# arneschneuing/DiffSBDD

Measured on AMD Instinct MI355X. Metric: sampled ligands/sec (500-step DDPM, fullatom_cond) at 1/2/4/8 MI355X, higher is better.
Workload: dtype f32

## Files before the change

### diffsbdd_amd/csrc/engine_state.h

```cpp
#pragma once

static thread_local std::string g_err;
static int fail(int code, const std::string& msg) { g_err = msg; return code; }

#define HIP_TRY(expr)                                                              \
  do {                                                                             \
    hipError_t _e = (expr);                                                        \
    if (_e != hipSuccess)                                                          \
      return fail(DSBDD_ERR_LAUNCH, std::string(#expr) + ": " + hipGetErrorString(_e)); \
  } while (0)
#define RC_TRY(expr)                       \
  do {                                     \
    const int _rc = (expr);                \
    if (_rc != DSBDD_OK) return _rc;       \
  } while (0)

struct StreamDevice {
  int prev = -1;
  bool switched = false;
  explicit StreamDevice(void* stream) {
    hipStream_t s = static_cast<hipStream_t>(stream);
    if (!s) return;
    hipDevice_t d = 0;
    int cur = 0;
// ... 113 lines not shown
  dsbdd_config cfg;
  std::vector<const float*> slots;
  bool has_weights = false;
  char* ws = nullptr;
  size_t ws_bytes = 0;
  int64_t cap_lig = 0, cap_poc = 0, cap_batch = 0, cap_edges = 0;
  bool lvl_stats_zeroed = false;
  int64_t cap_edgesL = 0;
  int prune = 1;
  int cone = 1;
  int64_t ghost_slots = 0;
  std::vector<int> plan_radius, plan_ghost;
  int plan_timed_level = kLevels - 1;
  bool frame = false;
  int64_t frame_nlig = 0, frame_npoc = 0, frame_batch = 0, frame_n3 = 0, frame_cap3 = 0;
  bool ghost_dirty = true;
  bool h0_pocket_valid = false;
  int64_t cap_tiles = 0;
  int64_t cap_tiles16 = 0;
  unsigned granule16 = 0;
  unsigned splitk = 0;
  int emu = 0;
  DerivedReady derived;
  float *trace_h = nullptr, *trace_x = nullptr;
  int n_cu = 256;
  int chain = 1;
  int64_t chain_min_rows = 0;
  int fork_front = 0;
  hipStream_t side_stream = nullptr;
  hipEvent_t ev_fork = nullptr, ev_join = nullptr;
  int level_rows = 0;
  int fold_scan = 1;
  int lig_head = 1;
  int edge_bperm = 1;
  int profile = 0;
  int64_t prof_call = 0;
  bool time_now = false;
  std::vector<hipEvent_t> ev;
  size_t ev_used = 0;
  struct GraphEntry {
    std::vector<uint64_t> key;
    int seen = 0;
    hipGraph_t graph = nullptr;
    hipGraphExec_t exec = nullptr;
    std::vector<int> plan_radius, plan_ghost;
    int plan_timed_level = 0;
    void destroy() { if (exec) (void)hipGraphExecDestroy(exec); if (graph) (void)hipGraphDestroy(graph); }
  };
  std::vector<GraphEntry> graphs;
  int use_graph = 1;
  int coord_split = 1;
  int node_group = 1;
  int edge_max_wg = 0;
  int64_t n_replay = 0, n_capture = 0, n_eager = 0;
  unsigned long long* ts_buf = nullptr;
  int ts_cap = 0, ts_next = 0;
  hipStream_t cap_stream = nullptr;
  dsbdd_engine() : Workspace{} {}
  void drop_graphs() {
    for (GraphEntry& g : graphs) g.destroy();
    graphs.clear();
  }
  void invalidate_derived() { derived = DerivedReady{}; }
  ~dsbdd_engine() {
    for (hipEvent_t e : ev) (void)hipEventDestroy(e);
    drop_graphs();
// ... 34 lines not shown
}
static int w2_pack_missing(dsbdd_engine* e, hipStream_t s) {
  const dsbdd_config& c = e->cfg;
  for (int kind = W2_KINDS - 1; kind >= 0; --kind) {
    if (!w2_enabled(e, kind) || e->derived.w2[kind]) continue;
    for (int blk = 0; blk < c.n_layers; ++blk)
      for (int which = 0; which < c.inv_sublayers + 2; ++which) {
        const float* src = which < c.inv_sublayers ? e->slots[gcl_slot(c, blk, which, DSBDD_GCL_E2_WT)]
                         : e->slots[eq_slot(c, blk, which == c.inv_sublayers ? DSBDD_EQ_C_W2T : DSBDD_EQ_X_W2T)];
        if (!src) continue;
        kW2Kinds[kind].pack(s, src, w2_copy(e, kind, blk, which), c.hidden_nf);
        HIP_TRY(hipGetLastError());
      }
    e->derived.w2[kind] = true;
  }
  return DSBDD_OK;
}

static bool env_int(const char* name, long long* v, bool mask = false) {
  const char* s = getenv(name);
  if (!s) return false;
  *v = mask ? (long long)strtoul(s, nullptr, 0) : (long long)atoi(s);
  return true;
}
static int env_int_in(const char* name, long long lo, long long hi, int dflt) {
  long long v;
  return env_int(name, &v) && v >= lo && v <= hi ? (int)v : dflt;
}
static void read_env_switches(dsbdd_engine* e) {
  long long v;
  const std::pair<const char*, int*> off_on_zero[] = {
      {"DSBDD_GRAPH", &e->use_graph}, {"DSBDD_EDGE_BPERM", &e->edge_bperm}, {"DSBDD_COORD_SPLIT", &e->coord_split},
      {"DSBDD_NODE_GROUP", &e->node_group}, {"DSBDD_PRUNE", &e->prune}, {"DSBDD_LIG_HEAD", &e->lig_head},
      {"DSBDD_NODE_CHAIN", &e->chain}};
  for (const auto& sw : off_on_zero) if (env_int(sw.first, &v) && v == 0) *sw.second = 0;
  const std::pair<const char*, int*> on_nonzero[] = {{"DSBDD_LEVEL_ROWS", &e->level_rows}, {"DSBDD_FORK", &e->fork_front}};
  for (const auto& sw : on_nonzero) if (env_int(sw.first, &v)) *sw.second = v != 0;
  if (env_int("DSBDD_FOLD_SCAN", &v)) e->fold_scan = v > 0 ? 1 : 0;
  if (env_int("DSBDD_GRANULE16", &v, true)) e->granule16 = (unsigned)v;
  if (env_int("DSBDD_SPLITK", &v, true)) e->splitk = (unsigned)v;
  if (env_int("DSBDD_EMU", &v)) e->emu = (v == 6 || v == 9) ? (int)v : 0;
  if (env_int("DSBDD_CONE", &v)) e->cone = v <= 0 ? 0 : (v >= 2 ? 2 : 1);
  if (env_int("DSBDD_NODE_CHAIN_MIN_ROWS", &v) && v >= 0) e->chain_min_rows = v;
  if (env_int("DSBDD_EDGE_MAX_WG", &v) && v > 0) e->edge_max_wg = (int)v;
}
```

### diffsbdd_amd/csrc/forward.h

```cpp
#pragma once

struct ForwardArgs {
  const float *xh_lig, *xh_pocket, *t;
  int64_t t_count;
  const int64_t *mask_lig, *mask_pocket;
  int64_t n_lig, n_pocket, batch;
  const int32_t *ext_row, *ext_col;
  int64_t ext_n_edges;
  float *eps_lig, *eps_pocket;
  int32_t* status;
};

static bool frame_applies(const dsbdd_engine* e, const ForwardArgs& a) {
  return e->frame && !e->cfg.update_pocket_coords && !a.ext_row && a.n_lig == e->frame_nlig &&
         a.n_pocket == e->frame_npoc && a.batch == e->frame_batch;
}

static Mlp2Problem residue_encoder(const dsbdd_engine* e, const ForwardArgs& a) {
  const dsbdd_config& c = e->cfg;
  const int r = c.residue_nf, J = c.joint_nf, JP = pad4(J + 1);
  const float* const* W = e->slots.data();
  return Mlp2Problem{a.xh_pocket + 3, 3 + r, r, W[DSBDD_G_RES_ENC_W0T], pad4(2 * r), W[DSBDD_G_RES_ENC_B0], 2 * r,
                     W[DSBDD_G_RES_ENC_W1T], pad4(J), W[DSBDD_G_RES_ENC_B1], J, e->h0 + (size_t)a.n_lig * JP, JP,
                     (int)a.n_pocket};
// ... 141 lines not shown
      }
    }
    HIP_TRY(nl(sa, e->h0, JP, JP, nullptr, 0, 0, W[DSBDD_G_EMB_WT], H, W[DSBDD_G_EMB_B], nullptr, 0, e->h, H, N, H, 0));
    if (split0) {
      hipLaunchKernelGGL(gather_rows_kernel, dim3((e->frame_n3 + 3) / 4), dim3(kThreads), 0, sa, e->h + (size_t)N * H,
                         (const float*)(e->h + (size_t)nlig * H), (const int*)e->frame_rows, (int)e->frame_n3, H);
      HIP_TRY(hipGetLastError());
    }
    if (fork) HIP_TRY(hipEventRecord(e->ev_join, sa));
    return DSBDD_OK;
  }

  int edge_list() {
    if (ext) {
      HIP_TRY(zero_async(e->deg, (size_t)N * 4, s));
      if (ext_n_edges > 0) {
        hipLaunchKernelGGL(ext_edges_kernel, dim3((int)((ext_n_edges + 255) / 256)), dim3(256), 0, s, ext_row,
                           ext_col, (int)ext_n_edges, (const float*)e->x, e->erow, e->ecol, e->ed0, e->deg);
        HIP_TRY(hipGetLastError());
      }
      hipLaunchKernelGGL(scan_kernel, dim3(1), dim3(1024), 0, s, (const int*)e->deg, e->row_ptr, N, SegAlign{},
                         (const int*)nullptr, (int*)nullptr, SegAlign{});
      HIP_TRY(hipGetLastError());
      edge_bound = ext_n_edges > 0 ? ext_n_edges : 1;
      if (subset) {
        hipLaunchKernelGGL(ext_flags_init_kernel, dim3((N + 255) / 256), dim3(256), 0, s, e->act_flag, nlig, N);
        HIP_TRY(hipGetLastError());
        if (ext_n_edges > 0) {
          hipLaunchKernelGGL(ext_flags_kernel, dim3((int)((ext_n_edges + 255) / 256)), dim3(256), 0, s, ext_row,
                             ext_col, (int)ext_n_edges, nlig, e->act_flag);
          HIP_TRY(hipGetLastError());
        }
      }
    } else {
      EdgeList2 l2{e->deg2, e->row_ptr2, e->erow2, e->ecol2, e->ed02, (int)e->cap_edges,
                   SegAlign{e->node_batch, e->lig_off, e->poc_off, nlig, B, e->scan_tmp2, e->seg_base2}};
      int rc = build_edges_impl(s, e->x, nlig, N, B, c, e->node_batch, e->lig_off, e->poc_off, e->deg,
                                e->row_ptr, e->erow, e->ecol, e->ed0, e->cap_edges, status,
                                subset ? e->act_flag : nullptr, e->scan_tmp, e->seg_base,
                                split0 ? &l2 : nullptr, 0, prune ? e->lvl : nullptr);
      if (rc) return rc;
      if (prune) {
        LevelArgs la{e->node_batch, e->lig_off, e->poc_off, nlig, B, e->lvl, e->deg, e->row_ptr, e->erow, e->ecol,
                     e->ed0, e->seg_rows, e->seg_edges, e->node_base, e->edge_base, e->lvl_cnt, e->lvl_end,
                     e->lvl_list, e->row_ptrL, e->erowL, e->ecolL, e->ed0L, (int)e->cap_edgesL, e->lvl_stats,
                     n_ghost, (int)ghost_slots, (int)e->cap_edges, nullptr, nullptr};
        mean_in_levels = e->fold_scan && n_mlp == 2;
        if (mean_in_levels) { la.mean_x = e->x; la.mean_out = e->mean; }
        if (!e->lvl_stats_zeroed) {
          HIP_TRY(zero_async(e->lvl_stats, 128, s));
          e->lvl_stats_zeroed = true;
        }
        hipLaunchKernelGGL(levels_kernel, dim3(B), dim3(kThreads), 0, s, la);
        HIP_TRY(hipGetLastError());
        if (!e->fold_scan) {
          hipLaunchKernelGGL(level_scan_kernel, dim3(1), dim3(1024), 0, s, la, N);
          HIP_TRY(hipGetLastError());
        }
        hipLaunchKernelGGL(level_place_kernel, dim3(B), dim3(kThreads), 0, s, la, e->fold_scan ? 1 : 0);
        HIP_TRY(hipGetLastError());
        int64_t cb = (e->cap_edges + 255) / 256;
        if (cb > 2048) cb = 2048;
        if (cb < 1) cb = 1;
        hipLaunchKernelGGL(level_copy_kernel, dim3((int)cb), dim3(256), 0, s, la, N);
        HIP_TRY(hipGetLastError());
      }
// ... 218 lines not shown
    const bool csk = ((e->splitk >> (16 + (blk & 15))) & 1u) && can_sk;
    const bool c16 = ((e->granule16 >> (16 + (blk & 15))) & 1u) && !e->emu && !csk;
    ea.xagg_stride = (size_t)N * 3; ea.xhead_stride = (size_t)(c16 ? e->cap_tiles16 : e->cap_tiles) * 4;
    ea.tile_ctr = e->tile_ctr; ea.norm_factor = c.normalization_factor;
    ea.pass_split = (c16 || csk) ? 1 : e->coord_split;
    if (e->ts_buf && e->ts_next < e->ts_cap) ea.ts = e->ts_buf + (size_t)(e->ts_next++) * 1024;
    HIP_TRY(launch_edge(e, s, MODE_COORD, ea, L_bound(), c16, csk));
    const int n_q = ((e->coord_split || c16 || csk) && n_mlp == 2) ? 2 : 1;
    const int c_shift = c16 ? 4 : 5, c_max = (int)(c16 ? e->cap_tiles16 : e->cap_tiles) - 1;
    const bool next_mean = subset && n_mlp == 2 && blk + 1 < c.n_layers;
    if (!subset) {
      if (n_upd > 0) {
        hipLaunchKernelGGL(coord_update_kernel, dim3((3 * n_upd + 255) / 256), dim3(256), 0, s, e->x,
                           (const float*)e->xagg, (const float*)e->xagg_head, n_q, ea.xagg_stride, ea.xhead_stride,
                           L_ptr, (const int*)e->deg, 3 * n_upd, c_max, c_shift);
        HIP_TRY(hipGetLastError());
      }
    } else if (n_upd > 0 || next_mean) {
      hipLaunchKernelGGL(coord_update_mean_kernel, dim3(B), dim3(kThreads), 0, s, e->x, (const float*)e->xagg,
                         (const float*)e->xagg_head, n_q, ea.xagg_stride, ea.xhead_stride, L_ptr,
                         (const int*)e->deg, n_upd, (const int*)e->lig_off, (const int*)e->poc_off, nlig,
                         next_mean ? e->mean : (float*)nullptr, c_max, c_shift);
      HIP_TRY(hipGetLastError());
    }
    return DSBDD_OK;
  }

  int output_head() {
    LigHeadArgs lh{e->h, H, W[DSBDD_G_EMBOUT_WT], JP, W[DSBDD_G_EMBOUT_B], J,
                   W[DSBDD_G_ATOM_DEC_W0T], pad4(2 * a), W[DSBDD_G_ATOM_DEC_B0], 2 * a,
                   W[DSBDD_G_ATOM_DEC_W1T], pad4(a), W[DSBDD_G_ATOM_DEC_B1], a,
                   e->x, e->x_in, nlig, N, eps_lig, dl, status};
    if (e->lig_head && !eps_pocket && !c.update_pocket_coords && lig_head_fits(lh)) {
      HIP_TRY(launch_lig_head(s, lh));
      return DSBDD_OK;
    }
    HIP_TRY(nl(s, e->h, H, H, nullptr, 0, 0, W[DSBDD_G_EMBOUT_WT], JP, W[DSBDD_G_EMBOUT_B], nullptr, 0, e->hout, JP,
               eps_pocket ? N : n_lig, JP, 0));
    {
      Mlp2Problem dec[2] = {
          {e->hout, JP, J, W[DSBDD_G_ATOM_DEC_W0T], pad4(2 * a), W[DSBDD_G_ATOM_DEC_B0], 2 * a,
           W[DSBDD_G_ATOM_DEC_W1T], pad4(a), W[DSBDD_G_ATOM_DEC_B1], a, eps_lig + 3, dl, (int)n_lig},
          {e->hout + (size_t)n_lig * JP, JP, J, W[DSBDD_G_RES_DEC_W0T], pad4(2 * r), W[DSBDD_G_RES_DEC_B0], 2 * r,
           W[DSBDD_G_RES_DEC_W1T], pad4(r), W[DSBDD_G_RES_DEC_B1], r, eps_pocket ? eps_pocket + 3 : nullptr, dp,
           (int)n_pocket}};
      if (mlp2_fits(dec[0]) && mlp2_fits(dec[1])) {
        HIP_TRY(launch_mlp2(s, dec, eps_pocket ? 2 : 1));
      } else {
        HIP_TRY(nl(s, e->hout, JP, J, nullptr, 0, 0, W[DSBDD_G_ATOM_DEC_W0T], pad4(2 * a), W[DSBDD_G_ATOM_DEC_B0], nullptr, 0,
                   e->enc_tmp, LE, n_lig, 2 * a, 1));
        HIP_TRY(nl(s, e->enc_tmp, LE, 2 * a, nullptr, 0, 0, W[DSBDD_G_ATOM_DEC_W1T], pad4(a), W[DSBDD_G_ATOM_DEC_B1], nullptr, 0,
                   eps_lig + 3, dl, n_lig, a, 0));
        if (eps_pocket) {
          float* tmp_p = e->enc_tmp + (size_t)n_lig * LE;
          HIP_TRY(nl(s, e->hout + (size_t)n_lig * JP, JP, J, nullptr, 0, 0, W[DSBDD_G_RES_DEC_W0T], pad4(2 * r),
                     W[DSBDD_G_RES_DEC_B0], nullptr, 0, tmp_p, LE, n_pocket, 2 * r, 1));
          HIP_TRY(nl(s, tmp_p, LE, 2 * r, nullptr, 0, 0, W[DSBDD_G_RES_DEC_W1T], pad4(r), W[DSBDD_G_RES_DEC_B1], nullptr, 0,
                     eps_pocket + 3, dp, n_pocket, r, 0));
        }
      }
    }
    hipLaunchKernelGGL(finalize_kernel, dim3(B), dim3(kThreads), 0, s, (const float*)e->x, (const float*)e->x_in,
                       (const int*)e->lig_off, (const int*)e->poc_off, nlig, c.update_pocket_coords, eps_lig, dl,
                       eps_pocket, dp, status);
    HIP_TRY(hipGetLastError());
    return DSBDD_OK;
  }
// ... 28 lines not shown
```

### diffsbdd_amd/csrc/graph.h

```cpp
#pragma once
#include "common.h"

namespace dsbdd {

constexpr int kTileCtrInts = 32;
constexpr int kEdgeAlign = 32;
constexpr int kLevels = 5;

struct Cutoffs {
  int has_l, has_p, has_i;
  float cl, cp, ci;
};

__device__ __forceinline__ int lower_bound_i64(const int64_t* a, int n, int64_t v) {
  int lo = 0, hi = n;
  while (lo < hi) {
    const int mid = (lo + hi) >> 1;
    if (a[mid] < v) lo = mid + 1; else hi = mid;
  }
  return lo;
}

__global__ void prep_kernel(const int64_t* mask_lig, int n_lig, const int64_t* mask_poc, int n_poc,
                            int B, int* node_batch, int* lig_off, int* poc_off, int* tile_ctr) {
// ... 178 lines not shown
    } else {
#pragma unroll
      for (int k = 0; k < 4; ++k) if (i0 + k < n) { out[i0 + k] = run; run += v[k]; }
    }
    carry += tile_total;
    __syncthreads();
  }
  if (t == 0) out[n] = carry;
  if (!seg.seg_base) return;
  __syncthreads();
  const int S = 2 * seg.B;
  auto seg_begin = [&](int k) { return k < seg.B ? seg.lig_off[k] : seg.n_lig + seg.poc_off[k - seg.B]; };
  auto seg_end = [&](int k) { return k < seg.B ? seg.lig_off[k + 1] : seg.n_lig + seg.poc_off[k - seg.B + 1]; };
  carry = 0;
  for (int base = 0; base < S; base += 1024) {
    const int k = base + t;
    int len = 0;
    if (k < S) len = (max(out[seg_end(k)] - out[seg_begin(k)], 0) + kEdgeAlign - 1) & ~(kEdgeAlign - 1);
    const int ex = carry + block_scan_1024(len, s_wave, s_carry_p);
    if (k < S) seg.seg_base[k] = ex;
    carry += s_carry;
    __syncthreads();
  }
  if (t == 0) {
    seg.seg_base[S] = carry;
    row_ptr[n] = carry;
  }
}

__device__ __forceinline__ void sample_mean_body(const float* x, const int* lig_off, const int* poc_off, int n_lig,
                                                 float* mean, float (*red)[kThreads]) {
  const int b = blockIdx.x, t = threadIdx.x;
  const int l0 = lig_off[b], l1 = lig_off[b + 1], p0 = n_lig + poc_off[b], p1 = n_lig + poc_off[b + 1];
  float s0 = 0.f, s1 = 0.f, s2 = 0.f;
  for (int i = l0 + t; i < l1; i += kThreads) { s0 += x[3 * i]; s1 += x[3 * i + 1]; s2 += x[3 * i + 2]; }
  for (int i = p0 + t; i < p1; i += kThreads) { s0 += x[3 * i]; s1 += x[3 * i + 1]; s2 += x[3 * i + 2]; }
  red[0][t] = s0; red[1][t] = s1; red[2][t] = s2;
  __syncthreads();
  for (int o = kThreads / 2; o > 0; o >>= 1) {
    if (t < o) { red[0][t] += red[0][t + o]; red[1][t] += red[1][t + o]; red[2][t] += red[2][t + o]; }
    __syncthreads();
  }
  if (t < 3) {
    int cnt = (l1 - l0) + (p1 - p0);
    if (cnt == 0) cnt = 1;
    mean[3 * b + t] = red[t][0] / (float)cnt;
  }
  __syncthreads();
}

struct LevelArgs {
  const int* node_batch; const int* lig_off; const int* poc_off; int n_lig; int B;
  int* lvl;
  const int* deg;
  const int* row_ptr_nat;
  const int* erow_nat; const int* ecol_nat; const float* ed0_nat;
  int* seg_rows;
  int* seg_edges;
  int* node_base;
  int* edge_base;
  int* lvl_cnt;
  int* lvl_end;
  int* lvl_list;
  int* row_ptr;
  int* erow; int* ecol; float* ed0; int e_cap;
  unsigned long long* stats;
  int node_off; int edge_off;
  int e_cap_nat;
  const float* mean_x; float* mean_out;
};
// ... 120 lines not shown
    for (int i = l0 + lane; i < l1; i += 64) {
      a.lvl_list[nb + (i - l0)] = i;
      a.row_ptr[i] = eb + (a.row_ptr_nat[i] - s0);
    }
    pads(eb + a.seg_edges[b]);
  }
  const int L = w + 1;
  if (L >= kLevels) return;
  const int p0 = a.n_lig + a.poc_off[b], p1 = a.n_lig + a.poc_off[b + 1];
  int n_run, e_run;
  if (fold_scan) level_bases(a, L * a.B + b, lane, n_run, e_run);
  else { n_run = a.node_base[L * a.B + b]; e_run = a.edge_base[L * a.B + b]; }
  for (int i0 = p0; i0 < p1; i0 += 64) {
    const int i = i0 + lane;
    const bool mine = i < p1 && a.lvl[i] == L;
    const int d = mine ? a.deg[i] : 0;
    const unsigned long long m = __ballot(mine);
    int incl = d;
#pragma unroll
    for (int o = 1; o < 64; o <<= 1) {
      const int u = __shfl_up(incl, o);
      if (lane >= o) incl += u;
    }
    if (mine) {
      a.lvl_list[n_run + __popcll(m & ((1ull << lane) - 1ull))] = i;
      a.row_ptr[i] = e_run + incl - d;
    }
    n_run += __popcll(m);
    e_run += __shfl(incl, 63);
  }
  pads(e_run);
}

__global__ void ghost_setup_kernel(const int* erow3, const int* ecol3, const float* ed03, const int* row_ptr3,
                                   const int* deg3, int n3, int id_src, int id_dst, int* erow, int* ecol,
                                   float* ed0, int e_cap, int* deg, int* row_ptr, int* lvl_list,
                                   const float* xframe, float* x) {
  const int total = min(row_ptr3[n3], e_cap);
  for (int p = blockIdx.x * blockDim.x + threadIdx.x; p < total; p += gridDim.x * blockDim.x) {
    const int r = erow3[p];
    erow[p] = r < 0 ? -1 : r - id_src + id_dst;
    ecol[p] = r < 0 ? 0 : ecol3[p] - id_src + id_dst;
    ed0[p] = ed03[p];
  }
  for (int i = blockIdx.x * blockDim.x + threadIdx.x; i < n3; i += gridDim.x * blockDim.x) {
    deg[id_dst + i] = deg3[i];
    row_ptr[id_dst + i] = row_ptr3[i];
    lvl_list[i] = id_dst + i;
    x[3 * (id_dst + i)] = xframe[3 * i]; x[3 * (id_dst + i) + 1] = xframe[3 * i + 1];
    x[3 * (id_dst + i) + 2] = xframe[3 * i + 2];
  }
}

__global__ __launch_bounds__(kThreads) void gather_rows_kernel(float* dst, const float* src, const int* rows, int n,
                                                               int H) {
  const int i = (blockIdx.x * kThreads + threadIdx.x) >> 6, lane = threadIdx.x & 63;
  if (i >= n) return;
  const float* a = src + (size_t)rows[i] * H;
  float* b = dst + (size_t)i * H;
  for (int k = 4 * lane; k < H; k += 256) *reinterpret_cast<float4*>(b + k) = ld4(a + k);
}

__global__ __launch_bounds__(kThreads) void canon_fill_kernel(float* h, const int* lvl, const int* twin_local,
                                                              int n_lig, int n_nodes, int ghost_base, int lo,
                                                              int hi, int H, float* pq = nullptr, int ldpq = 0) {
  const int i = n_lig + ((blockIdx.x * kThreads + threadIdx.x) >> 6), lane = threadIdx.x & 63;
// ... 221 lines not shown
```

### diffsbdd_amd/csrc/lig_head.h

```cpp
#pragma once
#include "common.h"

namespace dsbdd {

struct LigHeadArgs {
  const float* h; int H;
  const float* WoT; int ldo; const float* bo; int J;
  const float* W0T; int ld0; const float* b0; int n_hid;
  const float* W1T; int ld1; const float* b1; int n_out;
  const float* x; const float* x_in; int n_lig; int n_nodes;
  float* eps_lig; int dl; int* status;
};

constexpr int kHeadRows = 16;
constexpr int kHeadKC = 32;

__global__ __launch_bounds__(kThreads) void lig_head_kernel(LigHeadArgs p) {
  __shared__ __attribute__((aligned(16))) float sH[kHeadRows * 256];
  __shared__ float sO[kHeadRows * 128];
  __shared__ float sW[kHeadKC * 128];
  __shared__ float sD[kHeadRows * 64];
  const int t = threadIdx.x;
  const int r0 = blockIdx.x * kHeadRows;
  const int nr = min(kHeadRows, p.n_lig - r0);
// ... 53 lines not shown
    if (r >= nr) continue;
    float a = 0.f;
    for (int j = 0; j < p.n_hid; ++j) a = fmaf(sD[r * 64 + j], p.W1T[(size_t)j * p.ld1 + c], a);
    p.eps_lig[(size_t)(r0 + r) * p.dl + 3 + c] = a + p.b1[c];
  }
  bool nan = false;
  if (t < 3 * nr) {
    const int r = t / 3, k = t - 3 * r;
    const float v = p.x[3 * (size_t)(r0 + r) + k] - p.x_in[3 * (size_t)(r0 + r) + k];
    nan = v != v;
    p.eps_lig[(size_t)(r0 + r) * p.dl + k] = v;
  }
  {
    const int n_poc3 = 3 * (p.n_nodes - p.n_lig);
    const int per = (n_poc3 + gridDim.x - 1) / gridDim.x;
    const int lo = 3 * p.n_lig + blockIdx.x * per, hi = min(lo + per, 3 * p.n_nodes);
    for (int i = lo + t; i < hi; i += kThreads) {
      const float v = p.x[i] - p.x_in[i];
      nan = nan || (v != v);
    }
  }
  if (nan) atomicOr(p.status, 1);
}

inline bool lig_head_fits(const LigHeadArgs& a) {
  return a.H % kHeadKC == 0 && a.H <= 256 && a.J <= 128 && a.n_hid <= 64 && a.n_out <= 64 && a.n_lig > 0;
}

inline hipError_t launch_lig_head(hipStream_t s, const LigHeadArgs& a) {
  hipLaunchKernelGGL(lig_head_kernel, dim3((a.n_lig + kHeadRows - 1) / kHeadRows), dim3(kThreads), 0, s, a);
  return hipGetLastError();
}

}
```

Measured before the change: 38.69.

## Fuse per-sample edge build and level pruning into two front kernels; add lig_head2

Adds a per-sample path, used when pruning is on, that builds the radius graph in two block-per-sample kernels (count, then fill). The coordinates are staged in LDS, and level assignment, degree counting, segment prefix sums, level lists and padding are all computed in those kernels, replacing the longer sequence of build_edges and level kernels. It also adds a variant ligand output head that uses 8-row tiles, keeps the small MLP weights in LDS and register-prefetches the output weights. The aim is fewer launches and less global round-tripping per denoising step, at the cost of one block per sample with 1024 threads, which could underuse the GPU for small batches, and of heavy LDS use.

```diff
diff --git a/diffsbdd_amd/csrc/engine_state.h b/diffsbdd_amd/csrc/engine_state.h
--- a/diffsbdd_amd/csrc/engine_state.h
+++ b/diffsbdd_amd/csrc/engine_state.h
@@ -169,6 +169,8 @@
   int level_rows = 0;
   int fold_scan = 1;
   int lig_head = 1;
+  int front = 1;
+  int front_parts = 2;
   int edge_bperm = 1;
   int profile = 0;
   int64_t prof_call = 0;
@@ -269,11 +271,12 @@
   const std::pair<const char*, int*> off_on_zero[] = {
       {"DSBDD_GRAPH", &e->use_graph}, {"DSBDD_EDGE_BPERM", &e->edge_bperm}, {"DSBDD_COORD_SPLIT", &e->coord_split},
       {"DSBDD_NODE_GROUP", &e->node_group}, {"DSBDD_PRUNE", &e->prune}, {"DSBDD_LIG_HEAD", &e->lig_head},
-      {"DSBDD_NODE_CHAIN", &e->chain}};
+      {"DSBDD_NODE_CHAIN", &e->chain}, {"DSBDD_FRONT", &e->front}};
   for (const auto& sw : off_on_zero) if (env_int(sw.first, &v) && v == 0) *sw.second = 0;
   const std::pair<const char*, int*> on_nonzero[] = {{"DSBDD_LEVEL_ROWS", &e->level_rows}, {"DSBDD_FORK", &e->fork_front}};
   for (const auto& sw : on_nonzero) if (env_int(sw.first, &v)) *sw.second = v != 0;
   if (env_int("DSBDD_FOLD_SCAN", &v)) e->fold_scan = v > 0 ? 1 : 0;
+  if (env_int("DSBDD_FRONT_PARTS", &v, true)) e->front_parts = (int)(v & 3);
   if (env_int("DSBDD_GRANULE16", &v, true)) e->granule16 = (unsigned)v;
   if (env_int("DSBDD_SPLITK", &v, true)) e->splitk = (unsigned)v;
   if (env_int("DSBDD_EMU", &v)) e->emu = (v == 6 || v == 9) ? (int)v : 0;
diff --git a/diffsbdd_amd/csrc/forward.h b/diffsbdd_amd/csrc/forward.h
--- a/diffsbdd_amd/csrc/forward.h
+++ b/diffsbdd_amd/csrc/forward.h
@@ -197,6 +197,31 @@
           HIP_TRY(hipGetLastError());
         }
       }
+    } else if (prune && e->front && (e->front_parts & 1)) {
+      FrontArgs fa{};
+      fa.x = e->x; fa.n_nodes = N; fa.cut = cutoffs_of(c);
+      fa.deg = e->deg; fa.act_flag = e->act_flag;
+      fa.row_ptr = e->row_ptr; fa.erow = e->erow; fa.ecol = e->ecol; fa.ed0 = e->ed0; fa.e_cap = (int)e->cap_edges;
+      fa.seg_tot = e->node_base; fa.seg_base = e->seg_base;
+      if (split0)
+        fa.l2 = EdgeList2{e->deg2, e->row_ptr2, e->erow2, e->ecol2, e->ed02, (int)e->cap_edges,
+                          SegAlign{e->node_batch, e->lig_off, e->poc_off, nlig, B, e->scan_tmp2, e->seg_base2}};
+      fa.seg_tot2 = e->edge_base;
+      fa.lv = LevelArgs{e->node_batch, e->lig_off, e->poc_off, nlig, B, e->lvl, e->deg, e->row_ptr, e->erow, e->ecol,
+                        e->ed0, e->seg_rows, e->seg_edges, e->node_base, e->edge_base, e->lvl_cnt, e->lvl_end,
+                        e->lvl_list, e->row_ptrL, e->erowL, e->ecolL, e->ed0L, (int)e->cap_edgesL, e->lvl_stats,
+                        n_ghost, (int)ghost_slots, (int)e->cap_edges, nullptr, nullptr};
+      fa.status = status;
+      mean_in_levels = n_mlp == 2;
+      if (mean_in_levels) { fa.lv.mean_x = e->x; fa.lv.mean_out = e->mean; }
+      if (!e->lvl_stats_zeroed) {
+        HIP_TRY(zero_async(e->lvl_stats, 128, s));
+        e->lvl_stats_zeroed = true;
+      }
+      hipLaunchKernelGGL(front_count_kernel, dim3(B), dim3(kFrontThreads), 0, s, fa);
+      HIP_TRY(hipGetLastError());
+      hipLaunchKernelGGL(front_fill_kernel, dim3(B), dim3(kFrontThreads), 0, s, fa);
+      HIP_TRY(hipGetLastError());
     } else {
       EdgeList2 l2{e->deg2, e->row_ptr2, e->erow2, e->ecol2, e->ed02, (int)e->cap_edges,
                    SegAlign{e->node_batch, e->lig_off, e->poc_off, nlig, B, e->scan_tmp2, e->seg_base2}};
@@ -481,7 +506,7 @@
                    W[DSBDD_G_ATOM_DEC_W1T], pad4(a), W[DSBDD_G_ATOM_DEC_B1], a,
                    e->x, e->x_in, nlig, N, eps_lig, dl, status};
     if (e->lig_head && !eps_pocket && !c.update_pocket_coords && lig_head_fits(lh)) {
-      HIP_TRY(launch_lig_head(s, lh));
+      HIP_TRY(e->front && (e->front_parts & 2) && lig_head2_fits(lh) ? launch_lig_head2(s, lh) : launch_lig_head(s, lh));
       return DSBDD_OK;
     }
     HIP_TRY(nl(s, e->h, H, H, nullptr, 0, 0, W[DSBDD_G_EMBOUT_WT], JP, W[DSBDD_G_EMBOUT_B], nullptr, 0, e->hout, JP,
diff --git a/diffsbdd_amd/csrc/graph.h b/diffsbdd_amd/csrc/graph.h
--- a/diffsbdd_amd/csrc/graph.h
+++ b/diffsbdd_amd/csrc/graph.h
@@ -234,10 +234,12 @@
                                                  float* mean, float (*red)[kThreads]) {
   const int b = blockIdx.x, t = threadIdx.x;
   const int l0 = lig_off[b], l1 = lig_off[b + 1], p0 = n_lig + poc_off[b], p1 = n_lig + poc_off[b + 1];
-  float s0 = 0.f, s1 = 0.f, s2 = 0.f;
-  for (int i = l0 + t; i < l1; i += kThreads) { s0 += x[3 * i]; s1 += x[3 * i + 1]; s2 += x[3 * i + 2]; }
-  for (int i = p0 + t; i < p1; i += kThreads) { s0 += x[3 * i]; s1 += x[3 * i + 1]; s2 += x[3 * i + 2]; }
-  red[0][t] = s0; red[1][t] = s1; red[2][t] = s2;
+  if (t < kThreads) {
+    float s0 = 0.f, s1 = 0.f, s2 = 0.f;
+    for (int i = l0 + t; i < l1; i += kThreads) { s0 += x[3 * i]; s1 += x[3 * i + 1]; s2 += x[3 * i + 2]; }
+    for (int i = p0 + t; i < p1; i += kThreads) { s0 += x[3 * i]; s1 += x[3 * i + 1]; s2 += x[3 * i + 2]; }
+    red[0][t] = s0; red[1][t] = s1; red[2][t] = s2;
+  }
   __syncthreads();
   for (int o = kThreads / 2; o > 0; o >>= 1) {
     if (t < o) { red[0][t] += red[0][t + o]; red[1][t] += red[1][t + o]; red[2][t] += red[2][t + o]; }
@@ -424,6 +426,367 @@
   pads(e_run);
 }
 
+constexpr int kFrontThreads = 1024;
+constexpr int kFrontTile = 1024;
+
+struct FrontArgs {
+  const float* x; int n_nodes; Cutoffs cut;
+  int* deg; int* act_flag;
+  int* row_ptr; int* erow; int* ecol; float* ed0; int e_cap;
+  int* seg_tot; int* seg_base;
+  EdgeList2 l2; int* seg_tot2;
+  LevelArgs lv;
+  int* status;
+};
+
+struct FrontTileLds { float x[3 * kFrontTile]; int lvl[kFrontTile]; int deg[kFrontTile]; int deg2[kFrontTile]; };
+struct FrontPosLds { int nat[kFrontTile]; int two[kFrontTile]; int lev[kFrontTile]; };
+
+__device__ __forceinline__ int front_node(int c, int nl, int l0, int p0) { return c < nl ? l0 + c : p0 + (c - nl); }
+
+__device__ __forceinline__ void front_stage_x(FrontTileLds& T, const float* x, int nl, int np, int l0, int p0) {
+  const int n = min(nl + np, kFrontTile);
+  for (int c = threadIdx.x; c < n; c += kFrontThreads) {
+    const int j = front_node(c, nl, l0, p0);
+    T.x[3 * c] = x[3 * j]; T.x[3 * c + 1] = x[3 * j + 1]; T.x[3 * c + 2] = x[3 * j + 2];
+  }
+}
+
+__device__ __forceinline__ bool front_test(const FrontTileLds& T, const float* x, int c, int j, bool valid, float xi,
+                                           float yi, float zi, int has, float cutoff, float& d2) {
+  d2 = 0.f;
+  if (valid) {
+    float xj, yj, zj;
+    if (c < kFrontTile) { xj = T.x[3 * c]; yj = T.x[3 * c + 1]; zj = T.x[3 * c + 2]; }
+    else { xj = x[3 * j]; yj = x[3 * j + 1]; zj = x[3 * j + 2]; }
+    const float dx = xi - xj, dy = yi - yj, dz = zi - zj;
+    d2 = dx * dx + dy * dy + dz * dz;
+  }
+  return valid && (!has || __fsqrt_rn(d2) <= cutoff);
+}
+
+__device__ __forceinline__ int front_get(const int* tile, const int* glob, int c, int j) {
+  return c < kFrontTile ? tile[c] : glob[j];
+}
+__device__ __forceinline__ void front_row_x(const FrontTileLds& T, const float* x, int r, int i, float& xi, float& yi,
+                                            float& zi) {
+  if (r < kFrontTile) { xi = T.x[3 * r]; yi = T.x[3 * r + 1]; zi = T.x[3 * r + 2]; }
+  else { xi = x[3 * i]; yi = x[3 * i + 1]; zi = x[3 * i + 2]; }
+}
+__device__ __forceinline__ int front_lvl(const FrontTileLds& T, const int* lvl, int c, int j) {
+  return c < kFrontTile ? T.lvl[c] : lvl[j];
+}
+__device__ __forceinline__ void front_set_lvl(FrontTileLds& T, int* lvl, int c, int j, int v) {
+  lvl[j] = v;
+  if (c < kFrontTile) T.lvl[c] = v;
+}
+
+__global__ __launch_bounds__(kFrontThreads) void front_count_kernel(FrontArgs a) {
+  __shared__ FrontTileLds T;
+  __shared__ int s_rows[kLevels], s_edges[kLevels], s_nat[2], s_two[2];
+  __shared__ float s_red[3][kThreads];
+  const LevelArgs& v = a.lv;
+  if (v.mean_out) sample_mean_body(v.mean_x, v.lig_off, v.poc_off, v.n_lig, v.mean_out, s_red);
+  const int b = blockIdx.x, t = threadIdx.x, lane = t & 63, w = t >> 6;
+  constexpr int NW = kFrontThreads / 64;
+  const int l0 = v.lig_off[b], l1 = v.lig_off[b + 1];
+  const int p0 = v.n_lig + v.poc_off[b], p1 = v.n_lig + v.poc_off[b + 1];
+  const int nl = l1 - l0, np = p1 - p0, nc = nl + np;
+  const float* x = a.x;
+  if (t < kLevels) { s_rows[t] = 0; s_edges[t] = 0; }
+  if (t < 2) { s_nat[t] = 0; s_two[t] = 0; }
+  front_stage_x(T, x, nl, np, l0, p0);
+  __syncthreads();
+  for (int r = w; r < nc; r += NW) {
+    const int i = front_node(r, nl, l0, p0);
+    int L = 0;
+    if (r >= nl) {
+      float xi, yi, zi;
+      front_row_x(T, x, r, i, xi, yi, zi);
+      bool hit = false;
+      for (int c0 = 0; c0 < nl && !hit; c0 += 64) {
+        const int c = c0 + lane;
+        float d2;
+        hit = __ballot(front_test(T, x, c, l0 + c, c < nl, xi, yi, zi, a.cut.has_i, a.cut.ci, d2)) != 0ull;
+      }
+      L = hit ? 1 : kLevels - 1;
+    }
+    if (lane == 0) front_set_lvl(T, v.lvl, r, i, L);
+  }
+  __syncthreads();
+  for (int r = w; r < nc; r += NW) {
+    const int i = front_node(r, nl, l0, p0);
+    const bool il = r < nl;
+    float xi, yi, zi;
+    front_row_x(T, x, r, i, xi, yi, zi);
+    const bool far = !il && front_lvl(T, v.lvl, r, i) == kLevels - 1;
+    int cnt = 0, cnt_lig = 0;
+    bool near = false;
+#pragma unroll 1
+    for (int seg = 0; seg < 2; ++seg) {
+      const int c_begin = seg == 0 ? 0 : nl, c_end = seg == 0 ? nl : nc;
+      const bool jl = seg == 0;
+      const int has = (il && jl) ? a.cut.has_l : ((!il && !jl) ? a.cut.has_p : a.cut.has_i);
+      const float cu = (il && jl) ? a.cut.cl : ((!il && !jl) ? a.cut.cp : a.cut.ci);
+      for (int c0 = c_begin; c0 < c_end; c0 += 64) {
+        const int c = c0 + lane;
+        const bool valid = c < c_end;
+        const int j = front_node(c, nl, l0, p0);
+        float d2;
+        const bool pass = front_test(T, x, c, j, valid, xi, yi, zi, has, cu, d2);
+        cnt += __popcll(__ballot(pass));
+        if (far && !jl) near = near || (__ballot(pass && front_lvl(T, v.lvl, c, j) == 1) != 0ull);
+      }
+      if (seg == 0) cnt_lig = cnt;
+    }
+    if (lane == 0) {
+      a.deg[i] = cnt;
+      if (a.l2.deg) a.l2.deg[i] = il ? cnt : cnt_lig;
+      if (r < kFrontTile) { T.deg[r] = cnt; T.deg2[r] = il ? cnt : cnt_lig; }
+      if (a.act_flag) a.act_flag[i] = (il || cnt_lig > 0) ? 1 : 0;
+      if (near) front_set_lvl(T, v.lvl, r, i, 2);
+    }
+  }
+  for (int k = 3; k < kLevels - 1; ++k) {
+    __syncthreads();
+    for (int r = nl + w; r < nc; r += NW) {
+      const int i = p0 + (r - nl);
+      if (front_lvl(T, v.lvl, r, i) != kLevels - 1) continue;
+      float xi, yi, zi;
+      front_row_x(T, x, r, i, xi, yi, zi);
+      bool hit = false;
+      for (int c0 = nl; c0 < nc && !hit; c0 += 64) {
+        const int c = c0 + lane;
+        const int j = p0 + (c - nl);
+        float d2;
+        const bool pass = front_test(T, x, c, j, c < nc, xi, yi, zi, a.cut.has_p, a.cut.cp, d2);
+        hit = __ballot(pass && front_lvl(T, v.lvl, c, j) == k - 1) != 0ull;
+      }
+      if (hit && lane == 0) front_set_lvl(T, v.lvl, r, i, k);
+    }
+  }
+  __syncthreads();
+  for (int r = t; r < nc; r += kFrontThreads) {
+    const int i = front_node(r, nl, l0, p0);
+    const int L = r < nl ? 0 : front_lvl(T, v.lvl, r, i), d = front_get(T.deg, a.deg, r, i);
+    if (r >= nl) atomicAdd(&s_rows[L], 1);
+    atomicAdd(&s_edges[L], d);
+    atomicAdd(&s_nat[r < nl ? 0 : 1], d);
+    if (a.l2.deg) atomicAdd(&s_two[r < nl ? 0 : 1], front_get(T.deg2, a.l2.deg, r, i));
+  }
+  __syncthreads();
+  if (t < kLevels) {
+    v.seg_rows[t * v.B + b] = t == 0 ? nl : s_rows[t];
+    v.seg_edges[t * v.B + b] = s_edges[t];
+  }
+  if (t < 2) {
+    a.seg_tot[t * v.B + b] = s_nat[t];
+    if (a.l2.deg) a.seg_tot2[t * v.B + b] = s_two[t];
+  }
+}
+
+__device__ __forceinline__ int front_seg_prefix(const int* tot, int k, int lane) {
+  int s = 0;
+#pragma unroll 4
+  for (int k0 = 0; k0 < k; k0 += 64) {
+    const int kk = k0 + lane;
+    if (kk < k) s += (max(tot[kk], 0) + kEdgeAlign - 1) & ~(kEdgeAlign - 1);
+  }
+  return wave_sum_i(s);
+}
+
+__device__ __forceinline__ void front_level_bases(const LevelArgs& a, int k, int lane, int& nb, int& eb) {
+  int sn = 0, se = 0;
+#pragma unroll 4
+  for (int k0 = 0; k0 < k; k0 += 64) {
+    const int kk = k0 + lane;
+    if (kk < k) { sn += a.seg_rows[kk]; se += (a.seg_edges[kk] + kEdgeAlign - 1) & ~(kEdgeAlign - 1); }
+  }
+  nb = a.node_off + wave_sum_i(sn);
+  eb = a.edge_off + wave_sum_i(se);
+}
+
+__device__ __forceinline__ void front_seg_bases(const int* tot, int S, int lane, int* seg_base, int* total_out) {
+  int run = 0;
+  for (int k0 = 0; k0 < S; k0 += 64) {
+    const int kk = k0 + lane;
+    const int len = kk < S ? (max(tot[kk], 0) + kEdgeAlign - 1) & ~(kEdgeAlign - 1) : 0;
+    int incl = len;
+#pragma unroll
+    for (int o = 1; o < 64; o <<= 1) {
+      const int u = __shfl_up(incl, o);
+      if (lane >= o) incl += u;
+    }
+    if (kk < S) seg_base[kk] = run + incl - len;
+    run += __shfl(incl, 63);
+  }
+  if (lane == 0) { seg_base[S] = run; *total_out = run; }
+}
+
+__global__ __launch_bounds__(kFrontThreads) void front_fill_kernel(FrontArgs a) {
+  __shared__ FrontTileLds T;
+  __shared__ FrontPosLds P;
+  __shared__ int s_base[4 + 2 * kLevels];
+  const LevelArgs& v = a.lv;
+  const int b = blockIdx.x, t = threadIdx.x, lane = t & 63, w = t >> 6;
+  constexpr int NW = kFrontThreads / 64;
+  static_assert(NW >= 4 + kLevels + 3, "one wave per base / scan");
+  const int l0 = v.lig_off[b], l1 = v.lig_off[b + 1];
+  const int p0 = v.n_lig + v.poc_off[b], p1 = v.n_lig + v.poc_off[b + 1];
+  const int nl = l1 - l0, np = p1 - p0, nc = nl + np;
+  const float* x = a.x;
+  const bool two = a.l2.deg != nullptr;
+  front_stage_x(T, x, nl, np, l0, p0);
+  for (int c = t; c < min(nc, kFrontTile); c += kFrontThreads) {
+    const int j = front_node(c, nl, l0, p0);
+    T.lvl[c] = v.lvl[j]; T.deg[c] = a.deg[j]; T.deg2[c] = two ? a.l2.deg[j] : 0;
+  }
+  if (w < 2) {
+    const int s = front_seg_prefix(a.seg_tot, w * v.B + b, lane);
+    if (lane == 0) s_base[w] = s;
+  } else if (w < 4) {
+    const int s = two ? front_seg_prefix(a.seg_tot2, (w - 2) * v.B + b, lane) : 0;
+    if (lane == 0) s_base[w] = s;
+  } else if (w < 4 + kLevels) {
+    int nb, eb;
+    front_level_bases(v, (w - 4) * v.B + b, lane, nb, eb);
+    if (lane == 0) { s_base[w] = nb; s_base[w + kLevels] = eb; }
+  } else if (b == 0 && w == 4 + kLevels) {
+    unsigned long long ed_run = 0;
+    for (int q = 0; q < kLevels; ++q) {
+      int cn, ce;
+      front_level_bases(v, (q + 1) * v.B, lane, cn, ce);
+      int own = 0;
+      for (int k0 = q * v.B; k0 < (q + 1) * v.B; k0 += 64) { const int kk = k0 + lane; if (kk < (q + 1) * v.B) own += v.seg_edges[kk]; }
+      ed_run += (unsigned long long)wave_sum_i(own);
+      if (lane == 0) {
+        v.lvl_cnt[q] = cn; v.lvl_cnt[kLevels + q] = cn - v.node_off;
+        v.lvl_end[q] = ce; v.lvl_end[kLevels + q] = ce - v.edge_off;
+        if (v.stats) {
+          v.stats[q] += (unsigned long long)(cn - v.node_off);
+          v.stats[kLevels + q] += (unsigned long long)(ce - v.edge_off);
+          v.stats[2 * kLevels + q] += ed_run;
+          if (q == 0) v.stats[3 * kLevels] += 1ull;
+        }
+      }
+    }
+  } else if (b == 0 && w == 5 + kLevels) {
+    front_seg_bases(a.seg_tot, 2 * v.B, lane, a.seg_base, a.row_ptr + a.n_nodes);
+  } else if (b == 0 && w == 6 + kLevels && two) {
+    front_seg_bases(a.seg_tot2, 2 * v.B, lane, a.l2.seg.seg_base, a.l2.row_ptr + a.n_nodes);
+  }
+  __syncthreads();
+  auto pads = [&](int* er, int* ec, float* ed, int cap, int from) {
+    const int to = (from + kEdgeAlign - 1) & ~(kEdgeAlign - 1), pos = from + lane;
+    if (pos >= 0 && pos < to && pos < cap) { er[pos] = -1; ec[pos] = 0; ed[pos] = 0.f; }
+  };
+  auto wscan = [&](int d, int& tot) {
+    int incl = d;
+#pragma unroll
+    for (int o = 1; o < 64; o <<= 1) {
+      const int u = __shfl_up(incl, o);
+      if (lane >= o) incl += u;
+    }
+    tot = __shfl(incl, 63);
+    return incl - d;
+  };
+  if (w == 0) {
+    int run = 0;
+    for (int i0 = l0; i0 < l1; i0 += 64) {
+      const int i = i0 + lane;
+      const bool mine = i < l1;
+      int tot;
+      const int r = i - l0;
+      const int ex = run + wscan(mine ? front_get(T.deg, a.deg, r, i) : 0, tot);
+      if (mine) {
+        a.row_ptr[i] = s_base[0] + ex;
+        if (two) a.l2.row_ptr[i] = s_base[2] + ex;
+        v.row_ptr[i] = s_base[4 + kLevels] + ex;
+        v.lvl_list[s_base[4] + r] = i;
+        if (r < kFrontTile) { P.nat[r] = s_base[0] + ex; P.two[r] = s_base[2] + ex; P.lev[r] = s_base[4 + kLevels] + ex; }
+      }
+      run += tot;
+    }
+    pads(a.erow, a.ecol, a.ed0, a.e_cap, s_base[0] + run);
+    if (two) pads(a.l2.erow, a.l2.ecol, a.l2.ed0, a.l2.e_cap, s_base[2] + run);
+    pads(v.erow, v.ecol, v.ed0, v.e_cap, s_base[4 + kLevels] + run);
+  } else if (w < kLevels) {
+    const int L = w;
+    int n_run = s_base[4 + L], e_run = s_base[4 + kLevels + L];
+    for (int i0 = p0; i0 < p1; i0 += 64) {
+      const int i = i0 + lane;
+      const int r = nl + (i - p0);
+      const bool mine = i < p1 && front_get(T.lvl, v.lvl, r, i) == L;
+      const unsigned long long m = __ballot(mine);
+      int tot;
+      const int ex = wscan(mine ? front_get(T.deg, a.deg, r, i) : 0, tot);
+      if (mine) {
+        v.lvl_list[n_run + __popcll(m & ((1ull << lane) - 1ull))] = i;
+        v.row_ptr[i] = e_run + ex;
+        if (r < kFrontTile) P.lev[r] = e_run + ex;
+      }
+      n_run += __popcll(m);
+      e_run += tot;
+    }
+    pads(v.erow, v.ecol, v.ed0, v.e_cap, e_run);
+  } else if (w == kLevels || (w == kLevels + 1 && two)) {
+    const bool second = w == kLevels + 1;
+    const int* dg = second ? a.l2.deg : a.deg;
+    const int* dt = second ? T.deg2 : T.deg;
+    int* rp = second ? a.l2.row_ptr : a.row_ptr;
+    int* pt = second ? P.two : P.nat;
+    int run = s_base[second ? 3 : 1];
+    for (int i0 = p0; i0 < p1; i0 += 64) {
+      const int i = i0 + lane, r = nl + (i - p0);
+      int tot;
+      const int ex = wscan(i < p1 ? front_get(dt, dg, r, i) : 0, tot);
+      if (i < p1) {
+        rp[i] = run + ex;
+        if (r < kFrontTile) pt[r] = run + ex;
+      }
+      run += tot;
+    }
+    if (second) pads(a.l2.erow, a.l2.ecol, a.l2.ed0, a.l2.e_cap, run);
+    else pads(a.erow, a.ecol, a.ed0, a.e_cap, run);
+  }
+  __syncthreads();
+  for (int r = w; r < nc; r += NW) {
+    const int i = front_node(r, nl, l0, p0);
+    const bool il = r < nl;
+    float xi, yi, zi;
+    front_row_x(T, x, r, i, xi, yi, zi);
+    const int base = front_get(P.nat, a.row_ptr, r, i), base2 = two ? front_get(P.two, a.l2.row_ptr, r, i) : 0;
+    const int baseL = front_get(P.lev, v.row_ptr, r, i);
+    int cnt = 0;
+#pragma unroll 1
+    for (int seg = 0; seg < 2; ++seg) {
+      const int c_begin = seg == 0 ? 0 : nl, c_end = seg == 0 ? nl : nc;
+      const bool jl = seg == 0;
+      const int has = (il && jl) ? a.cut.has_l : ((!il && !jl) ? a.cut.has_p : a.cut.has_i);
+      const float cu = (il && jl) ? a.cut.cl : ((!il && !jl) ? a.cut.cp : a.cut.ci);
+      for (int c0 = c_begin; c0 < c_end; c0 += 64) {
+        const int c = c0 + lane;
+        const int j = front_node(c, nl, l0, p0);
+        float d2;
+        const bool pass = front_test(T, x, c, j, c < c_end, xi, yi, zi, has, cu, d2);
+        const unsigned long long m = __ballot(pass);
+        if (pass) {
+          const int k = cnt + __popcll(m & ((1ull << lane) - 1ull));
+          const int pos = base + k, posL = baseL + k;
+          if (pos >= 0 && pos < a.e_cap) { a.erow[pos] = i; a.ecol[pos] = j; a.ed0[pos] = d2; }
+          if (posL >= 0 && posL < v.e_cap) { v.erow[posL] = i; v.ecol[posL] = j; v.ed0[posL] = d2; }
+          if (two && (il || jl)) {
+            const int pos2 = base2 + k;
+            if (pos2 >= 0 && pos2 < a.l2.e_cap) { a.l2.erow[pos2] = i; a.l2.ecol[pos2] = j; a.l2.ed0[pos2] = d2; }
+          }
+        }
+        cnt += __popcll(m);
+      }
+    }
+    if (lane == 0 && base + cnt > a.e_cap) atomicOr(a.status, 2);
+  }
+}
+
 __global__ void ghost_setup_kernel(const int* erow3, const int* ecol3, const float* ed03, const int* row_ptr3,
                                    const int* deg3, int n3, int id_src, int id_dst, int* erow, int* ecol,
                                    float* ed0, int e_cap, int* deg, int* row_ptr, int* lvl_list,
diff --git a/diffsbdd_amd/csrc/lig_head.h b/diffsbdd_amd/csrc/lig_head.h
--- a/diffsbdd_amd/csrc/lig_head.h
+++ b/diffsbdd_amd/csrc/lig_head.h
@@ -109,4 +109,104 @@
   return hipGetLastError();
 }
 
-}
+constexpr int kHead2Rows = 8;
+constexpr int kHead2W0 = 4096;
+constexpr int kHead2W1 = 1024;
+
+__global__ __launch_bounds__(kThreads) void lig_head2_kernel(LigHeadArgs p) {
+  __shared__ __attribute__((aligned(16))) float sH[kHead2Rows * 256];
+  __shared__ float sO[kHead2Rows * 128];
+  __shared__ float sD[kHead2Rows * 64];
+  __shared__ float sW0[kHead2W0];
+  __shared__ float sW1[kHead2W1];
+  const int t = threadIdx.x;
+  const int r0 = blockIdx.x * kHead2Rows;
+  const int nr = min(kHead2Rows, p.n_lig - r0);
+  const int H = p.H, J = p.J;
+  for (int i = t; i < kHead2Rows * H / 4; i += kThreads) {
+    const int r = i / (H / 4), k4 = i - r * (H / 4);
+    float4 v = make_float4(0.f, 0.f, 0.f, 0.f);
+    if (r < nr) v = ld4(p.h + (size_t)(r0 + r) * H + 4 * k4);
+    *reinterpret_cast<float4*>(sH + r * H + 4 * k4) = v;
+  }
+  for (int i = t; i < J * p.ld0; i += kThreads) sW0[i] = i % p.ld0 < p.n_hid ? p.W0T[i] : 0.f;
+  for (int i = t; i < p.n_hid * p.ld1; i += kThreads) sW1[i] = i % p.ld1 < p.n_out ? p.W1T[i] : 0.f;
+  {
+    constexpr int RT = kHead2Rows / 2;
+    const int c = t & 127, rb = (t >> 7) * RT;
+    const float* wcol = p.WoT + (c < J ? c : 0);
+    float acc[RT];
+#pragma unroll
+    for (int i = 0; i < RT; ++i) acc[i] = 0.f;
+    float wn[8];
+#pragma unroll
+    for (int u = 0; u < 8; ++u) wn[u] = wcol[(size_t)u * p.ldo];
+    __syncthreads();
+    for (int k0 = 0; k0 < H; k0 += 8) {
+      float wv[8];
+#pragma unroll
+      for (int u = 0; u < 8; ++u) wv[u] = wn[u];
+      if (k0 + 8 < H) {
+#pragma unroll
+        for (int u = 0; u < 8; ++u) wn[u] = wcol[(size_t)(k0 + 8 + u) * p.ldo];
+      }
+#pragma unroll
+      for (int i = 0; i < RT; ++i) {
+        const float4 h0 = *reinterpret_cast<const float4*>(sH + (rb + i) * H + k0);
+        const float4 h1 = *reinterpret_cast<const float4*>(sH + (rb + i) * H + k0 + 4);
+        float a = acc[i];
+        a = fmaf(h0.w, wv[3], fmaf(h0.z, wv[2], fmaf(h0.y, wv[1], fmaf(h0.x, wv[0], a))));
+        a = fmaf(h1.w, wv[7], fmaf(h1.z, wv[6], fmaf(h1.y, wv[5], fmaf(h1.x, wv[4], a))));
+        acc[i] = a;
+      }
+    }
+    if (c < J) {
+      const float b = p.bo[c];
+#pragma unroll
+      for (int i = 0; i < RT; ++i) sO[(rb + i) * 128 + c] = acc[i] + b;
+    }
+  }
+  __syncthreads();
+  for (int idx = t; idx < kHead2Rows * p.n_hid; idx += kThreads) {
+    const int r = idx / p.n_hid, j = idx - r * p.n_hid;
+    float a = 0.f;
+    for (int k = 0; k < J; ++k) a = fmaf(sO[r * 128 + k], sW0[k * p.ld0 + j], a);
+    sD[r * 64 + j] = silu(a + p.b0[j]);
+  }
+  __syncthreads();
+  for (int idx = t; idx < kHead2Rows * p.n_out; idx += kThreads) {
+    const int r = idx / p.n_out, c = idx - r * p.n_out;
+    if (r >= nr) continue;
+    float a = 0.f;
+    for (int j = 0; j < p.n_hid; ++j) a = fmaf(sD[r * 64 + j], sW1[j * p.ld1 + c], a);
+    p.eps_lig[(size_t)(r0 + r) * p.dl + 3 + c] = a + p.b1[c];
+  }
+  bool nan = false;
+  if (t < 3 * nr) {
+    const int r = t / 3, k = t - 3 * r;
+    const float v = p.x[3 * (size_t)(r0 + r) + k] - p.x_in[3 * (size_t)(r0 + r) + k];
+    nan = v != v;
+    p.eps_lig[(size_t)(r0 + r) * p.dl + k] = v;
+  }
+  {
+    const int n_poc3 = 3 * (p.n_nodes - p.n_lig);
+    const int per = (n_poc3 + gridDim.x - 1) / gridDim.x;
+    const int lo = 3 * p.n_lig + blockIdx.x * per, hi = min(lo + per, 3 * p.n_nodes);
+    for (int i = lo + t; i < hi; i += kThreads) {
+      const float v = p.x[i] - p.x_in[i];
+      nan = nan || (v != v);
+    }
+  }
+  if (nan) atomicOr(p.status, 1);
+}
+
+inline bool lig_head2_fits(const LigHeadArgs& a) {
+  return lig_head_fits(a) && a.H % 8 == 0 && a.J * a.ld0 <= kHead2W0 && a.n_hid * a.ld1 <= kHead2W1;
+}
+
+inline hipError_t launch_lig_head2(hipStream_t s, const LigHeadArgs& a) {
+  hipLaunchKernelGGL(lig_head2_kernel, dim3((a.n_lig + kHead2Rows - 1) / kHead2Rows), dim3(kThreads), 0, s, a);
+  return hipGetLastError();
+}
+
+}
```

Result: no change. 38.81, median of 6 (+0.3%).
